# karenyang/GCN-VAE

Hardware: AMD Instinct MI355X
Metric: edges/sec R-GCN forward+backward, FB15k-237 emb=200 (higher is better)
Workload: dtype f32; 1 GPU; FB15k-237-shaped synthetic full graph (BASELINE configs[1]): 14541 entities, 474 directed relation types, E=544230 directed edges on this rank (544230 in the trained graph), 2-layer R-GCN-VAE bdd num_bases=100 emb_dim=200 dropout 0.2, 0 IAF blocks, DistMult decoder on T=220000 triplets per rank, step = fwd + loss(BCE+reg+KL+MMD) + bwd + clip + Adam; edges_per_gpu=544230, trained_graph_edges=544230, nodes=14541, triplets_per_gpu=220000, n_flows=0, gemm_precision=f32, launch=hipgraph, parallelism=single GPU, optimizer=replicated clip + Adam, k1_operands=f32

## Files before the change

### gcn-vae_amd/csrc/k_loss.hip

```cpp
#include "common.h"

namespace gv {

constexpr int RED_BLOCKS = 1024;

__device__ __forceinline__ float block_sum_256(float v, float* sm ) {
    v = wave_sum(v);
    const int lane = threadIdx.x & 63, w = threadIdx.x >> 6;
    __syncthreads();
    if (lane == 0) sm[w] = v;
    __syncthreads();
    return sm[0] + sm[1] + sm[2] + sm[3];
}

__global__ __launch_bounds__(256) void k_final_sum(const float* part, int n, float scale, float* out, int accumulate) {
    __shared__ float sm[4];
    float acc = 0.f;
    for (int i = threadIdx.x; i < n; i += 256) acc += part[i];
    const float tot = block_sum_256(acc, sm);
    if (threadIdx.x == 0) *out = accumulate ? *out + scale * tot : scale * tot;
}

__global__ __launch_bounds__(256) void k_loss_combine(const float* p0, int n0, float s0, const float* p1, int n1, float s1,
                                                      const float* p2, int n2, float s2, const float* p3, int n3, float s3,
// ... 984 lines not shown
    for (int g = 0; g < G; ++g) {
        float4 t;
        t.x = (rl_dyn(acc[g].x, l16) + rl_dyn(acc[g].x, 16 + l16)) + (rl_dyn(acc[g].x, 32 + l16) + rl_dyn(acc[g].x, 48 + l16));
        t.y = (rl_dyn(acc[g].y, l16) + rl_dyn(acc[g].y, 16 + l16)) + (rl_dyn(acc[g].y, 32 + l16) + rl_dyn(acc[g].y, 48 + l16));
        t.z = (rl_dyn(acc[g].z, l16) + rl_dyn(acc[g].z, 16 + l16)) + (rl_dyn(acc[g].z, 32 + l16) + rl_dyn(acc[g].z, 48 + l16));
        t.w = (rl_dyn(acc[g].w, l16) + rl_dyn(acc[g].w, 16 + l16)) + (rl_dyn(acc[g].w, 32 + l16) + rl_dyn(acc[g].w, 48 + l16));
        if (lane < 16) sm[w][l16 + 16 * g] = t;
    }
    __syncthreads();
    const bool indexed = !is_x && yidx;
    float* o = is_x ? gx + (size_t)row * h : gy + (size_t)(yidx ? yidx[row] : row) * h;
    for (int q = threadIdx.x; q < (h >> 2); q += 64 * MMD_WAVES) {
        float4 s4 = sm[0][q];
#pragma unroll
        for (int i = 1; i < MMD_WAVES; ++i) { const float4 t = sm[i][q]; s4.x += t.x; s4.y += t.y; s4.z += t.z; s4.w += t.w; }
        if (indexed) {
            atomicAdd(o + 4 * q, s4.x); atomicAdd(o + 4 * q + 1, s4.y); atomicAdd(o + 4 * q + 2, s4.z); atomicAdd(o + 4 * q + 3, s4.w);
        } else {
            *reinterpret_cast<float4*>(o + 4 * q) = s4;
        }
    }
}

__global__ __launch_bounds__(256) void k_prior_sample_fwd(const float* z_pre, const float* eps, float* out, int s, int k, int h) {
    const int total = s * h;
    for (int i = blockIdx.x * 256 + threadIdx.x; i < total; i += gridDim.x * 256) {
        const int r = i / h, c = i - r * h, j = r % k;
        const float v = softplus_t(z_pre[(size_t)(k + j) * h + c]) + 1e-8f;
        out[i] = z_pre[(size_t)j * h + c] + eps[i] * sqrtf(v);
    }
}

__global__ __launch_bounds__(256) void k_prior_sample_bwd(const float* z_pre, const float* eps, const float* g, float* gz_pre,
                                                          int accumulate, int s, int k, int h) {
    const int total = k * h;
    for (int i = blockIdx.x * 256 + threadIdx.x; i < total; i += gridDim.x * 256) {
        const int j = i / h, c = i - j * h;
        const float raw = z_pre[(size_t)(k + j) * h + c];
        const float v = softplus_t(raw) + 1e-8f;
        float gm = 0.f, gs = 0.f;
        for (int r = j; r < s; r += k) {
            gm += g[(size_t)r * h + c];
            gs += g[(size_t)r * h + c] * eps[(size_t)r * h + c];
        }
        const float gr = gs * 0.5f / sqrtf(v) * (raw > 20.f ? 1.f : 1.f / (1.f + expf(-raw)));
        gz_pre[i] = accumulate ? gz_pre[i] + gm : gm;
        gz_pre[total + i] = accumulate ? gz_pre[total + i] + gr : gr;
    }
}

struct DmFusedParams {
    const int4* items;
    int n_items;
    const int* rel_s;
    const int* rel_o;
    const int* rel_tid;
    const float* e;
    int ld_e;
    const float* w;
    int ld_w;
    const float* labels;
    const float* bias;
    const int* pos3;
    float* score;
    float* delta;
    float* u;
    float* partial;
    float* part;
    int h;
};

// ... 476 lines not shown
    static const int v2 = getenv("GV_MMD_ROWS16") ? atoi(getenv("GV_MMD_ROWS16")) : 1;
    const bool al = h % 4 == 0 && aligned16(x) && aligned16(y) && aligned16(gx) && aligned16(gy);
    if (v2 && al && h <= 256) hipLaunchKernelGGL(k_mmd_bwd_g<4>, dim3(sx + sy), dim3(64 * MMD_WAVES), 0, GV_ST, x, y, y_index, sx, sy, h, gmmd, gscale, gx, gy);
    else if (h <= 256) hipLaunchKernelGGL(k_mmd_bwd<4>, dim3(sx + sy), dim3(64 * MMD_WAVES), 0, GV_ST, x, y, y_index, sx, sy, h, gmmd, gscale, gx, gy);
    else hipLaunchKernelGGL(k_mmd_bwd<16>, dim3(sx + sy), dim3(64 * MMD_WAVES), 0, GV_ST, x, y, y_index, sx, sy, h, gmmd, gscale, gx, gy);
    return launch_status("gv_mmd_bwd");
}

extern "C" int gv_prior_sample_fwd(const float* z_pre, const float* eps, float* out, int s, int k, int h, void* stream) {
    GV_REQUIRE(z_pre && eps && out, GV_ERR_NULL, "gv_prior_sample_fwd: NULL pointer");
    GV_REQUIRE(s > 0 && k > 0 && h > 0, GV_ERR_SHAPE, "gv_prior_sample_fwd: bad shape");
    hipLaunchKernelGGL(k_prior_sample_fwd, dim3((s * h + 255) / 256), dim3(256), 0, GV_ST, z_pre, eps, out, s, k, h);
    return launch_status("gv_prior_sample_fwd");
}

extern "C" int gv_prior_sample_bwd(const float* z_pre, const float* eps, const float* g, float* gz_pre, int accumulate,
                                   int s, int k, int h, void* stream) {
    GV_REQUIRE(z_pre && eps && g && gz_pre, GV_ERR_NULL, "gv_prior_sample_bwd: NULL pointer");
    GV_REQUIRE(s > 0 && k > 0 && h > 0, GV_ERR_SHAPE, "gv_prior_sample_bwd: bad shape");
    hipLaunchKernelGGL(k_prior_sample_bwd, dim3((k * h + 255) / 256), dim3(256), 0, GV_ST, z_pre, eps, g, gz_pre, accumulate, s, k, h);
    return launch_status("gv_prior_sample_bwd");
}

extern "C" int gv_distmult_bce_fwd_grad(const int32_t* items, int n_items, const int32_t* rel_s, const int32_t* rel_o,
                                        const int32_t* rel_tid, const float* embed, int ld_e, const float* w_rel, int ld_w,
                                        const float* labels, const float* bias, const int32_t* pos3, float* score,
                                        float* delta, float* u, float* partial, float* workspace, int64_t t, int h,
                                        void* stream) {
    GV_REQUIRE(items && rel_s && rel_o && rel_tid && embed && w_rel && labels && score && delta && u && workspace,
               GV_ERR_NULL, "gv_distmult_bce_fwd_grad: NULL pointer");
    GV_REQUIRE(t > 0 && t < (1ll << 30) && n_items > 0, GV_ERR_SHAPE, "gv_distmult_bce_fwd_grad: t=%lld n_items=%d",
               (long long)t, n_items);
    GV_REQUIRE(h > 0 && h <= 256 && h % 4 == 0 && ld_e >= h && ld_w >= h && ld_e % 4 == 0 && ld_w % 4 == 0, GV_ERR_SHAPE,
               "gv_distmult_bce_fwd_grad: h=%d (ld %d, %d): the fused sweep covers h <= 256, h %% 4 == 0", h, ld_e, ld_w);
    GV_REQUIRE(aligned16(embed) && aligned16(w_rel) && aligned16(u) && aligned16(partial), GV_ERR_ALIGN,
               "gv_distmult_bce_fwd_grad: 16-B alignment required");
    DmFusedParams p{(const int4*)items, n_items, rel_s, rel_o, rel_tid, embed, ld_e, w_rel, ld_w, labels, bias, pos3,
                    score, delta, u, partial, workspace, h};
    hipLaunchKernelGGL(k_distmult_bce_fwd_grad<8>, dim3(red_blocks(t, 16)), dim3(256), 0, GV_ST, p);
    return launch_status("gv_distmult_bce_fwd_grad");
}

extern "C" int gv_distmult_grad_finish(const float* gloss, const float* u, const float* partial, const int32_t* fix,
                                       int n_fix, const int32_t* rowptr, int chunk, int num_rels, int h,
                                       const float* w_rel, int ld_w, float reg_scale, float* grad_w, int ld_gw,
                                       int accumulate, const float* delta, float* d_out, int64_t n_coef,
// ... 19 lines not shown
```

### gcn-vae_amd/encoders.py

```python
import random

import numpy as np
import torch
import torch.nn as nn
import torch.nn.functional as F

from . import ops, prob
from .flows import MADE, PermuteLayer
from .layers import RelGraphConv


class EmbeddingLayer(ops.StayOnDevice, nn.Module):
    def __init__(self, num_nodes, h_dim):
        super().__init__()
        self.embedding = nn.Embedding(num_nodes, h_dim)

    def forward(self, g, h, r, norm):
        h = ops.to_module_device(self.embedding.weight, h)
        return ops.embedding(self.embedding.weight, h.squeeze(), ops.device_rng(self.embedding.weight.device),
                             sole_consumer=True)


class DistLayer(ops.StayOnDevice, nn.Module):

# ... 49 lines not shown
        self.input_layer = EmbeddingLayer(self.num_nodes, self.h_dim)
        self.rconv_layer_1 = RelGraphConv(self.h_dim, self.h_dim, self.num_rels, "bdd", self.num_bases,
                                          activation=nn.ReLU(), self_loop=True, dropout=self.dropout)
        self.rconv_layer_2 = RelGraphConv(self.h_dim, self.h_dim * 2, self.num_rels, "bdd", self.num_bases,
                                          activation=None, self_loop=True, dropout=self.dropout)

    def sample_z(self, batch):
        m, v = prob.gaussian_parameters(self.z_pre.squeeze(0), dim=0)
        idx = torch.distributions.categorical.Categorical(self.pi).sample((batch,))
        x = prob.sample_gaussian(m[idx], v[idx])
        if self.n_flows > 0:
            for flow in self.nf[::-1]:
                x, _ = flow.inverse(x)
        return x

    def compute_kernel(self, x, y):
        dim = x.size(1)
        d2 = (x.unsqueeze(1) - y.unsqueeze(0)).pow(2).mean(2) / float(dim)
        return torch.exp(-d2)

    def get_kl(self, z):
        return ops.kl_to_mixture(z, self.z_mean, self.z_sigma, self.z_pre.squeeze(0), self.flow_log_prob)

    def _prior_draw(self, device, dtype):
        num_sample = 200
        rows = (num_sample // self.k) * self.k if num_sample // self.k > 1 else self.k
        if self.mmd_eps_override is not None:
            eps = self.mmd_eps_override
        elif self._prior_eps_next is not None:
            eps, self._prior_eps_next = self._prior_eps_next, None
        else:
            eps = torch.empty(rows, self.h_dim, device=device, dtype=dtype)
            ops.device_rng(device).fill([(eps, ops.RNG_NORMAL, 0.0, self.rng_stream_prior)])
        return ops.prior_sample(self.z_pre.squeeze(0), eps)

    def _prior_rows(self):
        num_sample = 200
        return (num_sample // self.k) * self.k if num_sample // self.k > 1 else self.k

    def _draw_noise(self, n, device):
        jobs, eps = [], self.eps_override
        for layer in (self.rconv_layer_1, self.rconv_layer_2):
            if layer.wants_keep_mask():
                layer._keep_next = torch.empty(n, layer.out_feat, dtype=torch.uint8, device=device)
                jobs.append(layer.keep_job(layer._keep_next))
        if eps is None:
            eps = torch.empty(n, self.h_dim, dtype=torch.float32, device=device)
            jobs.append((eps, ops.RNG_NORMAL, 0.0, self.rng_stream_eps))
        if self.batch_mmd_prior_with_forward and self.training and self.mmd_eps_override is None:
            self._prior_eps_next = torch.empty(self._prior_rows(), self.h_dim, dtype=torch.float32, device=device)
            jobs.append((self._prior_eps_next, ops.RNG_NORMAL, 0.0, self.rng_stream_prior))
        if jobs:
            ops.device_rng(device).fill(jobs)
        return eps

    def mmd_inputs(self, z):
        num_sample = 200
        if self._z_pri_flowed is not None:
            z_pri, self._z_pri_flowed = self._z_pri_flowed, None
        else:
            z_pri = self._prior_draw(z.device, z.dtype)
            if self.n_flows > 0:
                for flow in self.nf:
                    z_pri, _ = flow.forward(z_pri)
        if self.mmd_index_override is not None:
            pick = self.mmd_index_override
        elif self.row_part is not None and getattr(self.row_part, 'real_positions', None) is not None:
            real = self.row_part.real_positions
            pick = torch.as_tensor(real[random.sample(range(len(real)), num_sample)], device=z.device)
        else:
            pick = torch.tensor(random.sample(range(z.shape[0]), num_sample), device=z.device)
        return z_pri, pick

    def get_mmd(self, z):
        z_pri, pick = self.mmd_inputs(z)
        return ops.mmd(z_pri, ops.embedding(z, pick))

    def get_flow_log_prob(self):
        return self.flow_log_prob

    def _forward_rows(self, g, h, r, norm):
        from .distributed import AllGatherRows
        from .distributed import AllReduceSum
        part = self.row_part
# ... 130 lines not shown
```

### gcn-vae_amd/lib.py

```python
import ctypes
import os

import torch

_HERE = os.path.dirname(os.path.abspath(__file__))
LIB_PATH = os.path.join(_HERE, 'libgcnvae_hip.so')

_P, _I, _L, _F = ctypes.c_void_p, ctypes.c_int, ctypes.c_int64, ctypes.c_float

SIGNATURES = {
    'gv_version': (_I, []),
    'gv_last_error_string': (ctypes.c_char_p, []),
    'gv_index_caps': (None, [_L, _I, _I, _P, _P, _P]),
    'gv_index_workspace_bytes': (_L, [_L, _I]),
    'gv_build_csr': (_I, [_P, _L, _I, _I, _P, _P, _P, _I, _P, _I, _P, _L, _P]),
    'gv_build_csr_batch_workspace_bytes': (_L, [_P, _I]),
    'gv_build_csr_batch': (_I, [_P, _I, _P, _L, _P]),
    'gv_triplet_lists': (_I, [_P, _I, _L, _P, _P, _P, _P, _P, _P, _P, _P, _P]),
    'gv_widen2_i32': (_I, [_P, _P, _L, _P, _P, _L, _P]),
    'gv_graph_index_build': (_I, [_P, _P, _L, _I, _I, _I, _I, _P, _P, _P, _P, _I, _P, _I, _P, _P, _P, _P, _I, _P, _I, _P, _L, _P]),
    'gv_relation_index_build': (_I, [_P, _P, _P, _P, _P, _L, _I, _I, _P, _P, _P, _P, _P, _P, _P, _I, _P, _I, _P, _L, _P]),
    'gv_triplet_index_build': (_I, [_P, _L, _I, _I, _I, _I, _P, _P, _P, _P, _P, _I, _P, _I, _P, _P, _P, _P, _P, _I, _P, _I,
                                    _P, _L, _P]),
    'gv_perm_sample': (_I, [_L, _L, ctypes.c_uint64, ctypes.c_uint64, _P, _P, ctypes.c_uint32, _P, _P]),
# ... 107 lines not shown
    'gv_scatter_add_rows': (_I, [_P, _P, _P, _L, _I, _P]),
    'gv_reparam_fwd': (_I, [_P, _P, _P, _P, _P, _L, _I, _P]),
    'gv_reparam_bwd': (_I, [_P, _P, _P, _P, _P, _P, _P, _L, _I, _P]),
    'gv_distmult_bce_fwd': (_I, [_P, _I, _P, _I, _P, _P, _P, _P, _P, _P, _P, _L, _I, _P]),
    'gv_bce_grad': (_I, [_P, _P, _P, _P, _P, _P, _P, _P, _P, _L, _P]),
    'gv_distmult_bce_fwd_grad': (_I, [_P, _I, _P, _P, _P, _P, _I, _P, _I, _P, _P, _P, _P, _P, _P, _P, _P, _L, _I, _P]),
    'gv_distmult_grad_finish': (_I, [_P, _P, _P, _P, _I, _P, _I, _I, _I, _P, _I, _F, _P, _I, _I, _P, _P, _L, _P, _P, _L, _P]),
    'gv_mean_sq': (_I, [_P, _L, _F, _P, _P, _I, _P]),
    'gv_mean_sq2': (_I, [_P, _L, _F, _P, _L, _F, _P, _P, _P, _L, _P]),
    'gv_axpby': (_I, [_L, _P, _F, _P, _F, _P, _P]),
    'gv_mul': (_I, [_L, _P, _P, _P, _P]),
    'gv_mul_multi': (_I, [_I, _P, _P, _P, _P, _P]),
    'gv_kl_workspace_bytes': (_L, [_L, _I, _I]),
    'gv_kl_fwd': (_I, [_P, _P, _I, _P, _P, _P, _P, _P, _P, _L, _I, _I, _P, _P]),
    'gv_kl_bwd': (_I, [_P, _P, _I, _P, _P, _P, _P, _F, _F, _P, _P, _P, _P, _I, _P, _I, _L, _I, _I, _P, _P]),
    'gv_reparam_kl_fwd': (_I, [_P, _P, _P, _P, _P, _P, _P, _P, _L, _I, _I, _P]),
    'gv_reparam_kl_bwd': (_I, [_P, _P, _P, _P, _P, _P, _P, _F, _F, _P, _P, _P, _I, _P, _L, _I, _I, _P]),
    'gv_loss_combine': (_I, [_P, _L, _P, _L, _L, _P, _L, _I, _I, _P, _I, _I, _F, _F, _F, _P, _P, _P, _P]),
    'gv_lincomb4': (_I, [_P, _F, _P, _F, _P, _F, _P, _F, _P, _P]),
    'gv_mmd_fwd': (_I, [_P, _P, _P, _I, _I, _I, _P, _P, _P]),
    'gv_mmd_bwd': (_I, [_P, _P, _P, _I, _I, _I, _P, _F, _P, _P, _P]),
    'gv_prior_sample_fwd': (_I, [_P, _P, _P, _I, _I, _I, _P]),
    'gv_prior_sample_bwd': (_I, [_P, _P, _P, _P, _I, _I, _I, _I, _P]),
    'gv_iaf_update_fwd': (_I, [_P, _P, _I, _P, _P, _P, _L, _I, _P]),
    'gv_iaf_update_bwd': (_I, [_P, _P, _I, _P, _P, _P, _P, _P, _P, _L, _I, _P]),
    'gv_iaf_update_bwd_acc': (_I, [_P, _P, _I, _P, _P, _P, _P, _I, _P, _P, _L, _I, _P]),
    'gv_rowsum': (_I, [_P, _I, _I, _I, _P, _L, _P]),
    'gv_reverse_cols': (_I, [_P, _P, _L, _I, _P]),
    'gv_mean_rows_multi': (_I, [_I, _P, _L, _P, _P, _P, _P]),
    'gv_mean_rows_bwd': (_I, [_P, _L, _L, _P, _P, _P]),
    'gv_adam_step': (_I, [_P, _P, _P, _P, _L, _P, _F, _F, _F, _F, _F, _P, _P]),
    'gv_clip_adam_step': (_I, [_P, _P, _P, _P, _L, _P, _P, _F, _F, _F, _F, _F, _P, _I, _P]),
}

_lib = None
_fns = {}


def load():
    global _lib
    if _lib is None:
        if not os.path.exists(LIB_PATH):
            raise RuntimeError(
                f'{LIB_PATH} not found: the HIP extension is not built. Run `python gcn-vae_amd/_build.py` '
                '(or __graft_entry__.build()). There is no CPU fallback for this path.')
        lib = ctypes.CDLL(LIB_PATH)
# ... 53 lines not shown
```

### gcn-vae_amd/ops.py

```python
import contextlib
import ctypes as _ct
import itertools as _it
import os as _os
from dataclasses import dataclass
from typing import Optional

import torch

from . import lib
from .lib import ptr

ACT_NONE, ACT_RELU = 0, 1

DIRECT_GRAD = {}
GRAD_FRESH = set()
DIRECT_EPOCH = [0]


def _stamp_direct(ctx):
    ctx._gv_direct_epoch = DIRECT_EPOCH[0]


def _verify_direct(ctx):
    if getattr(ctx, '_gv_direct_epoch', DIRECT_EPOCH[0]) != DIRECT_EPOCH[0]:
# ... 2319 lines not shown
        out = torch.empty_like(eps)
        ctx.set_materialize_grads(False)
        lib.call('gv_prior_sample_fwd', ptr(z_pre), ptr(eps), ptr(out), eps.shape[0], k, h, lib.stream())
        ctx.save_for_backward(z_pre, eps)
        return out

    @staticmethod
    def backward(ctx, g):
        z_pre, eps = ctx.saved_tensors
        if g is None:
            return None, None
        g = _chk(g.contiguous(), name='g')
        d_zp = _direct_flat(z_pre)
        gz = d_zp if d_zp is not None else torch.empty_like(z_pre)
        lib.call('gv_prior_sample_bwd', ptr(z_pre), ptr(eps), ptr(g), ptr(gz), 1 if d_zp is not None else 0, eps.shape[0],
                 z_pre.shape[0] // 2, z_pre.shape[1], lib.stream())
        return (None if d_zp is not None else gz), None


def prior_sample(z_pre, eps):
    return _PriorSample.apply(z_pre, eps)


class _LossHead(torch.autograd.Function):

    @staticmethod
    def forward(ctx, z, z_mean, z_sigma, w_rel, z_pre, flp, z_pri, pick, labels, tidx, reg_w, kl_w, mmd_w, score_bias,
                embed_rows=None, rows_dev=None, kl_link=None, grad_mode=True):
        z, ld_z = _row_major(z, 'embed')
        if rows_dev is not None:
            rows_dev = _chk(rows_dev.reshape(-1), torch.int32, 'rows_dev')
            if kl_w <= 0 or embed_rows is not None:
                raise NotImplementedError('rows_dev needs kl_w > 0 (the padding rows are masked in the KL pass) and no embed_rows')
        w_rel, ld_w = _row_major(w_rel, 'w_relation')
        labels = _chk(labels.reshape(-1), name='labels')
        dev, (n, h), T = z.device, z.shape, tidx.T
        if labels.numel() != T:
            raise ValueError('labels / triplets length mismatch')
        f32 = dict(dtype=torch.float32, device=dev)
        ctx.set_materialize_grads(False)
        scal = torch.empty(4, **f32)
        pred, reg, kl, mmd = scal[0:1], scal[1:2], scal[2:3], scal[3:4]
        ws, ws2 = torch.empty(2048, **f32), torch.empty(1024, **f32)
        score = torch.empty(T, **f32)
        loss = torch.empty((), **f32)
        bias = flp if (score_bias and flp is not None) else None
        resp = wsk = z_post = wsm = None
        link = kl_link if (kl_link is not None and not kl_link.claimed and kl_w > 0 and flp is None and rows_dev is None
                           and embed_rows is None and kl_link.matches(z_pre) and kl_link.resp.shape[0] == n) else None
        if link is not None:
            link.claimed = True
        if kl_w > 0:
            z_mean, z_sigma = _chk(z_mean.contiguous(), name='z_mean'), _chk(z_sigma.contiguous(), name='z_sigma')
            z_pre = _chk(z_pre.contiguous(), name='z_pre')
            k = z_pre.shape[0] // 2
            if link is None:
                wsk = torch.empty(int(lib.load().gv_kl_workspace_bytes(n, h, k)) // 4, **f32)
                resp = torch.empty(n, k, **f32)
        if mmd_w > 0:
            z_pri = _chk(z_pri.contiguous(), name='z_pri')
            pick = _chk(pick.reshape(-1), torch.int64, 'pick')
            wsm = torch.empty(z_pri.shape[0] + pick.numel(), **f32)
        if ld_z != h or ld_w != h:
            raise ValueError('loss_head needs contiguous embeddings and relation table')
        st = lib.stream()
        if link is not None:
            resp, wsk = link.resp, link.ws
        elif kl_w > 0:
            lib.call('gv_kl_fwd', ptr(z), ptr(z_mean), h, ptr(z_sigma), ptr(z_pre), ptr(flp), ptr(resp), None, ptr(wsk),
                     n, h, k, ptr(rows_dev), st)
        if mmd_w > 0:
            lib.call('gv_mmd_fwd', ptr(z_pri), ptr(z), ptr(pick), z_pri.shape[0], pick.numel(), h, None, ptr(wsm), st)
        z_count = z.numel() if embed_rows is None else int(embed_rows) * h
        lib.call('gv_mean_sq2', ptr(z), z.numel(), 1.0 / z_count, ptr(w_rel), w_rel.numel(), 1.0 / w_rel.numel(), None,
                 ptr(ws2), ptr(rows_dev), n, st)
        ctx.fused = None
        if grad_mode and (ctx.needs_input_grad[0] or ctx.needs_input_grad[3]) and distmult_fused_ok(z, ld_z, w_rel, ld_w):
            ctx.fused = _distmult_fused_fwd(z, ld_z, w_rel, ld_w, labels, bias, tidx, score, ws)
            ctx.ws = ws
        else:
            lib.call('gv_distmult_bce_fwd', ptr(z), ld_z, ptr(w_rel), ld_w, ptr(tidx.trip32), ptr(tidx.fwd_order), ptr(labels),
                     ptr(bias), ptr(score), None, ptr(ws), T, h, st)
        lib.call('gv_loss_combine', ptr(ws), T, ptr(ws2), z.numel(), w_rel.numel(), ptr(wsk) if kl_w > 0 else None, n, h,
                 (z_pre.shape[0] // 2) if kl_w > 0 else 0, ptr(wsm) if mmd_w > 0 else None,
                 z_pri.shape[0] if mmd_w > 0 else 0, pick.numel() if mmd_w > 0 else 0, float(reg_w), float(kl_w),
                 float(mmd_w), ptr(scal), ptr(loss), ptr(rows_dev), st)
        ctx.save_for_backward(z, z_mean if kl_w > 0 else None, z_sigma if kl_w > 0 else None, w_rel,
                              z_pre if kl_w > 0 else None, resp, z_pri if mmd_w > 0 else None, z_post,
                              pick if mmd_w > 0 else None, labels, score, wsk, rows_dev)
        ctx.meta = (tidx, float(reg_w), float(kl_w), float(mmd_w), bias is not None, flp is not None and kl_w > 0)
        ctx.z_count = z_count
        ctx.kl_link = link
        ctx.direct_w = _direct(w_rel) if ld_w == h else None
        _stamp_direct(ctx)
        out_pred, out_kl, out_mmd = pred.reshape(()), kl.reshape(1), mmd.reshape(())
        ctx.mark_non_differentiable(out_pred, out_kl, out_mmd)
        return loss, out_pred, out_kl, out_mmd

    @staticmethod
    def backward(ctx, g, _gp, _gk, _gm):
        if g is None:
            return (None,) * 18
        z, z_mean, z_sigma, w_rel, z_pre, resp, z_pri, z_post, pick, labels, score, wsk, rows_dev = ctx.saved_tensors
        z_count = ctx.z_count
        tidx, reg_w, kl_w, mmd_w, has_bias, flp_in_kl = ctx.meta
        dev, (n, h), T = z.device, z.shape, tidx.T
        f32 = dict(dtype=torch.float32, device=dev)
        g = _chk(g.reshape(1).contiguous(), name='gloss')
        fused = ctx.fused
        dscore = torch.empty(T, **f32) if fused is None else None
        dbias = torch.empty((), **f32) if has_bias else None
        ws = torch.empty(1024, **f32) if fused is None else None
        link = ctx.kl_link
        gz = torch.empty_like(z) if link is None else None
        gm = gv = gzp = d_zp = g_pri = g_post = None
        if link is not None:
            link.gkl, link.gscale, link.z_extra = g, kl_w, 2.0 * reg_w / z_count
            d_zp = True
        elif kl_w > 0:
            k = z_pre.shape[0] // 2
            d_zp = _direct_flat(z_pre)
            gm, gv = torch.empty_like(z), torch.empty_like(z)
            gzp = d_zp if d_zp is not None else torch.empty_like(z_pre)
        if mmd_w > 0:
            g_pri = torch.empty_like(z_pri)
        _verify_direct(ctx)
        d_w = ctx.direct_w
        g_w = d_w if d_w is not None else torch.empty_like(w_rel)
        g_flp = torch.empty((), **f32) if (has_bias or flp_in_kl) else None
        st = lib.stream()
        with fork(1):
            s1 = lib.stream()
            if link is not None:
                pass
            elif kl_w > 0:
                lib.call('gv_kl_bwd', ptr(z), ptr(z_mean), h, ptr(z_sigma), ptr(z_pre), ptr(resp), ptr(g), kl_w,
                         2.0 * reg_w / z_count, ptr(gz), ptr(gm), ptr(gv), ptr(gzp), 1 if d_zp is not None else 0, ptr(wsk),
                         1, n, h, k, ptr(rows_dev), s1)
            else:
                lib.call('gv_axpby', z.numel(), ptr(g), 2.0 * reg_w / z_count, ptr(z), 0.0, ptr(gz), s1)
            if mmd_w > 0 and link is None:
                lib.call('gv_mmd_bwd', ptr(z_pri), ptr(z), ptr(pick), z_pri.shape[0], pick.numel(), h, ptr(g), mmd_w,
                         ptr(g_pri), ptr(gz), s1)
        if fused is not None:
            d_inc = _distmult_fused_finish(fused, g, tidx, w_rel, h, 2.0 * reg_w / w_rel.numel(), g_w, d_w is not None, ctx.ws,
                                           dbias)
            idx_inc = None if tidx.pos3 is not None else tidx.inc_tid
        else:
            if tidx.pos3 is not None:
                d_inc, d_rel, idx_inc, idx_rel = torch.empty(2 * T, **f32), torch.empty(T, **f32), None, None
            else:
                d_inc, d_rel, idx_inc, idx_rel = dscore, dscore, tidx.inc_tid, tidx.rel_tid
            lib.call('gv_bce_grad', ptr(score), ptr(labels), ptr(g), ptr(dscore), ptr(tidx.pos3),
                     ptr(d_inc) if tidx.pos3 is not None else None, ptr(d_rel) if tidx.pos3 is not None else None,
                     ptr(dbias), ptr(ws), T, st)
            bdd_grad_weight(tidx.rel, tidx.rel_s, tidx.rel_o, d_rel, idx_rel, z, z, h, 1, 1, out=g_w,
                            accumulate=d_w is not None)
            lib.call('gv_axpby', w_rel.numel(), ptr(g), 2.0 * reg_w / w_rel.numel(), ptr(w_rel), 1.0, ptr(g_w), st)
        join(1)
        g_z = bdd_aggregate(indices.largest_first(tidx.inc) if indices.K1_ITEMS_LARGEST_FIRST else tidx.inc, tidx.inc_other, tidx.inc_rel,
                            d_inc, idx_inc, z, w_rel, h, 1, 1, addend=gz)
        if link is not None and mmd_w > 0:
            lib.call('gv_mmd_bwd', ptr(z_pri), ptr(z), ptr(pick), z_pri.shape[0], pick.numel(), h, ptr(g), mmd_w,
                     ptr(g_pri), ptr(g_z), st)
        if g_flp is not None:
            lib.call('gv_lincomb4', ptr(dbias) if has_bias else None, 1.0, ptr(g) if flp_in_kl else None, kl_w, None, 0.0,
                     None, 0.0, ptr(g_flp), st)
        return (g_z, gm, gv, (None if d_w is not None else g_w), (None if d_zp is not None else gzp), g_flp, g_pri, None,
                None, None, None, None, None, None, None, None, None, None)


def loss_head(z, z_mean, z_sigma, w_rel, z_pre, flp, z_pri, pick, labels, tidx, reg_w, kl_w, mmd_w, score_bias,
              embed_rows=None, rows_dev=None):
    return _LossHead.apply(z, z_mean, z_sigma, w_rel, z_pre, flp, z_pri, pick, labels, tidx, float(reg_w), float(kl_w),
                           float(mmd_w), bool(score_bias), embed_rows, rows_dev, getattr(z, '_gv_kl_link', None),
                           torch.is_grad_enabled())


from .made import *
from .made import _ChainLayer, _RowLayer, _MADEForward, _MADEForwardBF16
from . import made


TRANSE_MAX_DIM = 512


def _i32(t, name, n=None):
    t = _chk(t, torch.int32, name)
    if not t.is_contiguous() or (n is not None and t.numel() != n):
        raise ValueError(f'{name}: expected a contiguous int32 tensor of {n} entries')
    return t


def _table(t, name):
    t = _chk(t, name=name)
    if t.dim() != 2 or not t.is_contiguous() or not 1 <= t.shape[1] <= TRANSE_MAX_DIM:
# ... 294 lines not shown
```

### gcn-vae_amd/train.py

```python
import argparse
import time

import numpy as np
import torch
import torch.nn as nn

from . import ops, ranking, sampling
from .optim import FlatAdam
from .data import load_data
from .encoders import KGVAE, RGCN
from .sampling import node_norm_to_edge_norm


class LinkPredict(ops.StayOnDevice, nn.Module):
    def __init__(self, model_class, in_dim, h_dim, num_rels, num_bases=-1, num_hidden_layers=1, dropout=0,
                 use_cuda=True, reg_param=0, kl_param=0, mmd_param=0, k=1, n_flows=0):
        super().__init__()
        self.encoder = model_class(num_nodes=in_dim, h_dim=h_dim, out_dim=h_dim, num_rels=num_rels * 2,
                                   num_bases=num_bases, num_hidden_layers=num_hidden_layers, dropout=dropout,
                                   use_self_loop=use_cuda, use_cuda=use_cuda, k=k, n_flows=n_flows)
        self.reg_param, self.kl_param, self.mmd_param = reg_param, kl_param, mmd_param
        if kl_param > 0 and hasattr(self.encoder, 'fuse_kl_with_reparam'):
            self.encoder.fuse_kl_with_reparam = True
        if mmd_param > 0 and hasattr(self.encoder, 'batch_mmd_prior_with_forward'):
# ... 8 lines not shown
        if key != self._tidx_key:
            self._tidx = ops.TripletIndex(triplets.to(embedding.device), embedding.shape[0], self.w_relation.shape[0],
                                          sync_free=not getattr(self, 'static_batch', False))
            self._tidx_key = key
            self._tidx_keepalive = triplets
        return self._tidx

    def calc_score(self, embedding, triplets):
        return ops.distmult_score(embedding, self.w_relation, self.triplet_index(embedding, triplets))

    def forward(self, g, h, r, norm):
        return self.encoder.forward(g, h, r, norm)

    def regularization_loss(self, embedding):
        return ops.mean_sq(embedding) + ops.mean_sq(self.w_relation)

    def get_loss(self, g, embed, triplets, labels):
        enc = self.encoder
        tidx = self.triplet_index(embed, triplets)
        vae = isinstance(enc, KGVAE)
        flp = enc.get_flow_log_prob() if vae else None
        kl_w = self.kl_param if vae else 0.0
        mmd_w = self.mmd_param if vae else 0.0
        z_pri, pick = enc.mmd_inputs(embed) if mmd_w > 0 else (None, None)
        part = getattr(enc, 'row_part', None) if vae else None
        if part is not None:
            return self._get_loss_rows(part, embed, tidx, flp, kl_w, mmd_w, z_pri, pick, labels)
        loss, predict_loss, kl, mmd = ops.loss_head(
            embed, enc.z_mean if kl_w > 0 else None, enc.z_sigma if kl_w > 0 else None, self.w_relation,
            enc.z_pre.squeeze(0) if kl_w > 0 else None, flp, z_pri, pick, labels, tidx, self.reg_param, kl_w, mmd_w,
            score_bias=self.n_flows > 0, rows_dev=getattr(self, 'rows_dev', None))
        kl = kl.reshape(()) if kl_w > 0 else kl.reshape(1)
        mmd = mmd.reshape(()) if mmd_w > 0 else mmd.reshape(1)
        if kl_w <= 0 or mmd_w <= 0:
            loss = loss.reshape(1)
        return loss, predict_loss, kl, mmd


def _get_loss_rows(self, part, embed, tidx, flp, kl_w, mmd_w, z_pri, pick, labels):
    enc = self.encoder
    head, predict_loss, _, mmd = ops.loss_head(embed, None, None, self.w_relation, None, flp, z_pri, pick, labels, tidx,
                                               self.reg_param, 0.0, mmd_w, score_bias=self.n_flows > 0,
                                               embed_rows=part.real_rows)
    kl = None
    if kl_w > 0 and part.own_rows > 0:
        kl = ops.kl_to_mixture(enc.z_own, enc.z_mean, enc.z_sigma, enc.z_pre.squeeze(0), flp)
    loss = ops.lincomb2(head, 1.0 / part.world, kl, kl_w * part.own_rows / max(part.real_rows, 1))
# ... 319 lines not shown
```

### include/gcnvae.h

```cpp
#ifndef GCNVAE_H
#define GCNVAE_H

#include <stdint.h>

#ifdef __cplusplus
extern "C" {
#endif

typedef enum {
    GV_OK = 0,
    GV_ERR_NULL = -1,
    GV_ERR_SHAPE = -2,
    GV_ERR_ALIGN = -3,
    GV_ERR_WORKSPACE = -4
} gv_status;

enum { GV_ACT_NONE = 0, GV_ACT_RELU = 1 };

int gv_version(void);
const char* gv_last_error_string(void);

int gv_segment_items_count(const int32_t* rowptr, int n_seg, int chunk, int32_t* n_chunks, int32_t* n_slots,
                           int32_t* is_split, void* stream);
int gv_segment_items_fill(const int32_t* rowptr, int n_seg, int chunk, const int32_t* item_off,
// ... 346 lines not shown
int gv_kl_bwd(const float* z, const float* m, int ld_m, const float* v, const float* z_pre, const float* resp,
              const float* gkl, float gscale, float z_extra, float* gz, float* gm, float* gv, float* g_zpre,
              int accumulate_zpre, float* workspace, int mix_ready, int64_t n, int h, int k, const int32_t* rows_dev,
              void* stream);
int gv_reparam_kl_fwd(const float* h2, const float* eps, const float* z_pre, float* z, float* v, float* m_out, float* resp,
                      float* workspace, int64_t n, int h, int k, void* stream);
int gv_reparam_kl_bwd(const float* z, const float* h2, const float* v, const float* eps, const float* z_pre, const float* resp,
                      const float* gkl, float gscale, float z_extra, const float* gz_up, float* gh2, float* g_zpre,
                      int accumulate_zpre, float* workspace, int64_t n, int h, int k, void* stream);

int gv_loss_combine(const float* ws_pred, int64_t t, const float* ws_reg, int64_t n_embed, int64_t n_wrel,
                    const float* ws_kl, int64_t n_nodes, int h, int k, const float* ws_mmd, int sx, int sy, float reg_w,
                    float kl_w, float mmd_w, float* scal , float* loss, const int32_t* rows_dev,
                    void* stream);
int gv_lincomb4(const float* a0, float c0, const float* a1, float c1, const float* a2, float c2, const float* a3,
                float c3, float* out, void* stream);
int gv_mmd_fwd(const float* x, const float* y, const int64_t* y_index, int sx, int sy, int h, float* mmd, float* workspace,
               void* stream);
int gv_mmd_bwd(const float* x, const float* y, const int64_t* y_index, int sx, int sy, int h, const float* gmmd, float gscale,
               float* gx, float* gy, void* stream);
int gv_prior_sample_fwd(const float* z_pre, const float* eps, float* out, int s, int k, int h, void* stream);
int gv_prior_sample_bwd(const float* z_pre, const float* eps, const float* g, float* gz_pre, int accumulate, int s, int k,
                        int h, void* stream);

int gv_iaf_update_fwd(const float* z, const float* net, int ld_net, const float* x_old, const int32_t* colcount,
                      float* x_new, int64_t n, int d, void* stream);
int gv_iaf_update_bwd(const float* z, const float* net, int ld_net, const int32_t* colcount, const float* g_xnew,
                      const float* g_logdet , float* g_z, float* g_net, float* g_xold, int64_t n, int d,
                      void* stream);
int gv_iaf_update_bwd_acc(const float* z, const float* net, int ld_net, const int32_t* colcount, const float* g_xnew,
                          const float* g_logdet, float* g_z, int gz_accumulate, float* g_net, float* g_xold, int64_t n, int d,
                          void* stream);
int gv_rowsum(const float* x, int ld, int col0, int ncols, float* out, int64_t n, void* stream);
int gv_reverse_cols(const float* x, float* out, int64_t n, int d, void* stream);
int gv_mean_rows_multi(int count, const float* const* x, int64_t n, const int32_t* rows_dev, float* out, float* workspace,
                       void* stream);
int gv_mean_rows_bwd(const float* g, int64_t len, int64_t n, const int32_t* rows_dev, float* out, void* stream);

int gv_adam_step(float* p, const float* g, float* exp_avg, float* exp_avg_sq, int64_t n, const float* sumsq,
                 float max_norm, float lr, float beta1, float beta2, float eps, const float* step, void* stream);
int gv_clip_adam_step(float* p, float* g, float* exp_avg, float* exp_avg_sq, int64_t n, float* workspace,
                      float* sumsq_out, float max_norm, float lr, float beta1, float beta2, float eps, float* step,
                      int zero_grad, void* stream);

void gv_index_caps(int64_t n_entries, int n_seg, int chunk, int* items_cap, int* fix_cap, int* slots_cap);
int64_t gv_index_workspace_bytes(int64_t n_entries, int n_seg_max);
// ... 63 lines not shown
```

Measured before the change: 569.4 million edges/s.

## Fuse prior sampling with MMD forward and gradient into one kernel pass

Defers the prior draw so that one kernel builds the prior samples from z_pre and eps and computes both the MMD value and per-row gradient directions in the forward pass. A small apply kernel then scales those directions by the upstream gradient and scatters them into the decoder and z_pre gradients. This removes the separate prior_sample forward/backward and MMD backward kernels and their passes over the pairwise rows. In exchange the forward always pays for the gradient work, adds buffers for u_pri and u_post, and only applies under a set of shape and alignment conditions.

```diff
diff --git a/gcn-vae_amd/csrc/k_loss.hip b/gcn-vae_amd/csrc/k_loss.hip
--- a/gcn-vae_amd/csrc/k_loss.hip
+++ b/gcn-vae_amd/csrc/k_loss.hip
@@ -1030,12 +1030,17 @@
     }
 }
 
+__device__ __forceinline__ float prior_sd(float raw) {
+    const float v = softplus_t(raw) + 1e-8f;
+    return sqrtf(v);
+}
+__device__ __forceinline__ float prior_elem(float mu, float e, float sd) { return mu + e * sd; }
+
 __global__ __launch_bounds__(256) void k_prior_sample_fwd(const float* z_pre, const float* eps, float* out, int s, int k, int h) {
     const int total = s * h;
     for (int i = blockIdx.x * 256 + threadIdx.x; i < total; i += gridDim.x * 256) {
         const int r = i / h, c = i - r * h, j = r % k;
-        const float v = softplus_t(z_pre[(size_t)(k + j) * h + c]) + 1e-8f;
-        out[i] = z_pre[(size_t)j * h + c] + eps[i] * sqrtf(v);
+        out[i] = prior_elem(z_pre[(size_t)j * h + c], eps[i], prior_sd(z_pre[(size_t)(k + j) * h + c]));
     }
 }
 
@@ -1055,6 +1060,145 @@
         gz_pre[i] = accumulate ? gz_pre[i] + gm : gm;
         gz_pre[total + i] = accumulate ? gz_pre[total + i] + gr : gr;
     }
+}
+
+template <int G>
+__global__ __launch_bounds__(64 * MMD_WAVES) void k_mmd_fwd_grad_g(const float* z_pre, const float* eps, int k, const float* y,
+                                                                    const int64_t* yidx, int sx, int sy, int h, float* z_pri,
+                                                                    float* part, float* u_pri, float* u_post) {
+    extern __shared__ __attribute__((aligned(16))) float4 smx[];
+    __shared__ float smt[MMD_WAVES];
+    const int lane = threadIdx.x & 63, l16 = lane & 15, w = threadIdx.x >> 6;
+    const int grp = (int)(threadIdx.x >> 4);
+    constexpr int NG = 4 * MMD_WAVES;
+    const int h4 = h >> 2, kh4 = k * h4;
+    float4* red = smx + 2 * kh4;
+    for (int i = threadIdx.x; i < kh4; i += 64 * MMD_WAVES) {
+        smx[i] = reinterpret_cast<const float4*>(z_pre)[i];
+        const float4 r4 = reinterpret_cast<const float4*>(z_pre)[kh4 + i];
+        smx[kh4 + i] = make_float4(prior_sd(r4.x), prior_sd(r4.y), prior_sd(r4.z), prior_sd(r4.w));
+    }
+    __syncthreads();
+    const bool is_x = (int)blockIdx.x < sx;
+    const int row = is_x ? blockIdx.x : blockIdx.x - sx;
+    bool on[G];
+    int col[G];
+#pragma unroll
+    for (int g = 0; g < G; ++g) { col[g] = 4 * (l16 + 16 * g); on[g] = col[g] < h; }
+    auto load_row = [&](bool from_y, int j, float4 (&v)[G]) {
+        if (from_y) {
+            mmd_load_row4<G>(y + (size_t)(yidx ? yidx[j] : j) * h, on, col, v);
+        } else {
+            const float* e = eps + (size_t)j * h;
+            const float4* mu = smx + (j % k) * h4;
+#pragma unroll
+            for (int g = 0; g < G; ++g) {
+                v[g] = make_float4(0.f, 0.f, 0.f, 0.f);
+                if (on[g]) {
+                    const float4 e4 = *reinterpret_cast<const float4*>(e + col[g]);
+                    const float4 m4 = mu[col[g] >> 2], s4 = mu[kh4 + (col[g] >> 2)];
+                    v[g] = make_float4(prior_elem(m4.x, e4.x, s4.x), prior_elem(m4.y, e4.y, s4.y), prior_elem(m4.z, e4.z, s4.z),
+                                       prior_elem(m4.w, e4.w, s4.w));
+                }
+            }
+        }
+    };
+    float4 av[G], acc[G];
+    load_row(!is_x, row, av);
+    if (is_x && threadIdx.x < 16) {
+#pragma unroll
+        for (int g = 0; g < G; ++g)
+            if (on[g]) *reinterpret_cast<float4*>(z_pri + (size_t)row * h + col[g]) = av[g];
+    }
+#pragma unroll
+    for (int g = 0; g < G; ++g) acc[g] = make_float4(0.f, 0.f, 0.f, 0.f);
+    const float inv = 1.f / ((float)h * (float)h);
+    const int n_same = is_x ? sx : sy, n_other = is_x ? sy : sx;
+    const float c_same = (-2.f * inv) * 2.f / ((float)n_same * (float)n_same);
+    const float c_other = (-2.f * inv) * (-2.f) / ((float)sx * (float)sy);
+    float tot = 0.f;
+    for (int pass = 0; pass < 2; ++pass) {
+        const bool b_is_y = pass == 0 ? !is_x : is_x;
+        const int nb = pass == 0 ? n_same : n_other;
+        const float cf = pass == 0 ? c_same : c_other;
+        const bool counts = pass == 0 || is_x;
+        const float wt = pass == 0 ? 1.f / ((float)nb * (float)nb) : -2.f / ((float)sx * (float)sy);
+        for (int j0 = 0; j0 < nb; j0 += 2 * NG) {
+            const int j = j0 + grp, j1 = j + NG;
+            float4 b0[G], b1[G];
+            load_row(b_is_y, min(j, nb - 1), b0);
+            load_row(b_is_y, min(j1, nb - 1), b1);
+            const float d0 = row16_sum(mmd_d2_4<G>(av, b0)), d1 = row16_sum(mmd_d2_4<G>(av, b1));
+            const float e0 = expf(-d0 * inv), e1 = expf(-d1 * inv);
+            if (counts) {
+                if (j < nb) tot += wt * e0;
+                if (j1 < nb) tot += wt * e1;
+            }
+            const float k0 = j < nb ? cf * e0 : 0.f, k1 = j1 < nb ? cf * e1 : 0.f;
+#pragma unroll
+            for (int g = 0; g < G; ++g) {
+                acc[g].x = fmaf(k0, av[g].x - b0[g].x, fmaf(k1, av[g].x - b1[g].x, acc[g].x));
+                acc[g].y = fmaf(k0, av[g].y - b0[g].y, fmaf(k1, av[g].y - b1[g].y, acc[g].y));
+                acc[g].z = fmaf(k0, av[g].z - b0[g].z, fmaf(k1, av[g].z - b1[g].z, acc[g].z));
+                acc[g].w = fmaf(k0, av[g].w - b0[g].w, fmaf(k1, av[g].w - b1[g].w, acc[g].w));
+            }
+        }
+    }
+    const float t = (rl_bcast_f(tot, 0) + rl_bcast_f(tot, 16)) + (rl_bcast_f(tot, 32) + rl_bcast_f(tot, 48));
+    if (lane == 0) smt[w] = t;
+#pragma unroll
+    for (int g = 0; g < G; ++g) {
+        float4 s;
+        s.x = (rl_dyn(acc[g].x, l16) + rl_dyn(acc[g].x, 16 + l16)) + (rl_dyn(acc[g].x, 32 + l16) + rl_dyn(acc[g].x, 48 + l16));
+        s.y = (rl_dyn(acc[g].y, l16) + rl_dyn(acc[g].y, 16 + l16)) + (rl_dyn(acc[g].y, 32 + l16) + rl_dyn(acc[g].y, 48 + l16));
+        s.z = (rl_dyn(acc[g].z, l16) + rl_dyn(acc[g].z, 16 + l16)) + (rl_dyn(acc[g].z, 32 + l16) + rl_dyn(acc[g].z, 48 + l16));
+        s.w = (rl_dyn(acc[g].w, l16) + rl_dyn(acc[g].w, 16 + l16)) + (rl_dyn(acc[g].w, 32 + l16) + rl_dyn(acc[g].w, 48 + l16));
+        if (lane < 16) red[w * 16 * G + l16 + 16 * g] = s;
+    }
+    __syncthreads();
+    if (threadIdx.x == 0) {
+        float s = 0.f;
+#pragma unroll
+        for (int i = 0; i < MMD_WAVES; ++i) s += smt[i];
+        part[blockIdx.x] = s;
+    }
+    float* o = (is_x ? u_pri : u_post) + (size_t)row * h;
+    for (int q = threadIdx.x; q < h4; q += 64 * MMD_WAVES) {
+        float4 s4 = red[q];
+#pragma unroll
+        for (int i = 1; i < MMD_WAVES; ++i) { const float4 x = red[i * 16 * G + q]; s4.x += x.x; s4.y += x.y; s4.z += x.z; s4.w += x.w; }
+        *reinterpret_cast<float4*>(o + 4 * q) = s4;
+    }
+}
+
+__global__ __launch_bounds__(256) void k_mmd_grad_apply(const float* u_pri, const float* u_post, const int64_t* pick,
+                                                        const float* z_pre, const float* eps, const float* gmmd, float gscale,
+                                                        float* gdec, int64_t n, float* gz_pre, int accumulate, int sx, int sy,
+                                                        int k, int h, int nb_post) {
+    const float c = gscale * (gmmd ? *gmmd : 1.f);
+    if ((int)blockIdx.x < nb_post) {
+        const int i = blockIdx.x * 256 + threadIdx.x;
+        if (i >= sy * h) return;
+        const int r = i / h, cc = i - r * h;
+        const int64_t dst = pick ? pick[r] : r;
+        if (dst >= 0 && dst < n) atomicAdd(gdec + dst * h + cc, c * u_post[i]);
+        return;
+    }
+    const int total = k * h;
+    const int i = ((int)blockIdx.x - nb_post) * 256 + threadIdx.x;
+    if (i >= total) return;
+    const int j = i / h, cc = i - j * h;
+    const float raw = z_pre[(size_t)(k + j) * h + cc];
+    const float v = softplus_t(raw) + 1e-8f;
+    float gm = 0.f, gs = 0.f;
+    for (int r = j; r < sx; r += k) {
+        const float g = c * u_pri[(size_t)r * h + cc];
+        gm += g;
+        gs += g * eps[(size_t)r * h + cc];
+    }
+    const float gr = gs * 0.5f / sqrtf(v) * (raw > 20.f ? 1.f : 1.f / (1.f + expf(-raw)));
+    gz_pre[i] = accumulate ? gz_pre[i] + gm : gm;
+    gz_pre[total + i] = accumulate ? gz_pre[total + i] + gr : gr;
 }
 
 struct DmFusedParams {
@@ -1577,6 +1721,34 @@
     return launch_status("gv_prior_sample_bwd");
 }
 
+extern "C" int gv_mmd_fused_ok(int h, int k) {
+    return h > 0 && k > 0 && h % 4 == 0 && h <= 256 && (int64_t)k * h <= 4096;
+}
+
+extern "C" int gv_mmd_fwd_grad(const float* z_pre, const float* eps, int k, const float* y, const int64_t* y_index, int sx, int sy,
+                               int h, float* z_pri, float* workspace, float* u_pri, float* u_post, void* stream) {
+    GV_REQUIRE(z_pre && eps && y && z_pri && workspace && u_pri && u_post, GV_ERR_NULL, "gv_mmd_fwd_grad: NULL pointer");
+    GV_REQUIRE(sx > 0 && sy > 0 && sx + sy <= RED_BLOCKS && gv_mmd_fused_ok(h, k), GV_ERR_SHAPE,
+               "gv_mmd_fwd_grad: sx=%d sy=%d h=%d k=%d (need h %% 4 == 0, h <= 256, k h <= 4096, sx+sy <= %d)", sx, sy, h, k, RED_BLOCKS);
+    GV_REQUIRE(aligned16(z_pre) && aligned16(eps) && aligned16(y) && aligned16(z_pri) && aligned16(u_pri) && aligned16(u_post),
+               GV_ERR_SHAPE, "gv_mmd_fwd_grad: rows must be 16-byte aligned");
+    const size_t lds = ((size_t)2 * k * (h / 4) + (size_t)MMD_WAVES * 16 * 4) * sizeof(float4);
+    hipLaunchKernelGGL(k_mmd_fwd_grad_g<4>, dim3(sx + sy), dim3(64 * MMD_WAVES), lds, GV_ST, z_pre, eps, k, y, y_index, sx, sy, h,
+                       z_pri, workspace, u_pri, u_post);
+    return launch_status("gv_mmd_fwd_grad");
+}
+
+extern "C" int gv_mmd_grad_apply(const float* u_pri, const float* u_post, const int64_t* pick, const float* z_pre, const float* eps,
+                                 const float* gmmd, float gscale, float* g_dec, int64_t n, float* gz_pre, int accumulate, int sx,
+                                 int sy, int k, int h, void* stream) {
+    GV_REQUIRE(u_pri && u_post && z_pre && eps && g_dec && gz_pre, GV_ERR_NULL, "gv_mmd_grad_apply: NULL pointer");
+    GV_REQUIRE(sx > 0 && sy > 0 && k > 0 && h > 0 && n > 0 && (pick || sy <= n), GV_ERR_SHAPE, "gv_mmd_grad_apply: bad shape");
+    const int nb_post = (sy * h + 255) / 256;
+    hipLaunchKernelGGL(k_mmd_grad_apply, dim3(nb_post + (k * h + 255) / 256), dim3(256), 0, GV_ST, u_pri, u_post, pick, z_pre, eps,
+                       gmmd, gscale, g_dec, n, gz_pre, accumulate, sx, sy, k, h, nb_post);
+    return launch_status("gv_mmd_grad_apply");
+}
+
 extern "C" int gv_distmult_bce_fwd_grad(const int32_t* items, int n_items, const int32_t* rel_s, const int32_t* rel_o,
                                         const int32_t* rel_tid, const float* embed, int ld_e, const float* w_rel, int ld_w,
                                         const float* labels, const float* bias, const int32_t* pos3, float* score,
diff --git a/gcn-vae_amd/encoders.py b/gcn-vae_amd/encoders.py
--- a/gcn-vae_amd/encoders.py
+++ b/gcn-vae_amd/encoders.py
@@ -95,7 +95,7 @@
     def get_kl(self, z):
         return ops.kl_to_mixture(z, self.z_mean, self.z_sigma, self.z_pre.squeeze(0), self.flow_log_prob)
 
-    def _prior_draw(self, device, dtype):
+    def _prior_draw(self, device, dtype, deferred=False):
         num_sample = 200
         rows = (num_sample // self.k) * self.k if num_sample // self.k > 1 else self.k
         if self.mmd_eps_override is not None:
@@ -105,7 +105,7 @@
         else:
             eps = torch.empty(rows, self.h_dim, device=device, dtype=dtype)
             ops.device_rng(device).fill([(eps, ops.RNG_NORMAL, 0.0, self.rng_stream_prior)])
-        return ops.prior_sample(self.z_pre.squeeze(0), eps)
+        return (ops.prior_draw if deferred else ops.prior_sample)(self.z_pre.squeeze(0), eps)
 
     def _prior_rows(self):
         num_sample = 200
@@ -127,12 +127,12 @@
             ops.device_rng(device).fill(jobs)
         return eps
 
-    def mmd_inputs(self, z):
+    def mmd_inputs(self, z, deferred=False):
         num_sample = 200
         if self._z_pri_flowed is not None:
             z_pri, self._z_pri_flowed = self._z_pri_flowed, None
         else:
-            z_pri = self._prior_draw(z.device, z.dtype)
+            z_pri = self._prior_draw(z.device, z.dtype, deferred and self.n_flows == 0)
             if self.n_flows > 0:
                 for flow in self.nf:
                     z_pri, _ = flow.forward(z_pri)
diff --git a/gcn-vae_amd/lib.py b/gcn-vae_amd/lib.py
--- a/gcn-vae_amd/lib.py
+++ b/gcn-vae_amd/lib.py
@@ -153,6 +153,9 @@
     'gv_mmd_bwd': (_I, [_P, _P, _P, _I, _I, _I, _P, _F, _P, _P, _P]),
     'gv_prior_sample_fwd': (_I, [_P, _P, _P, _I, _I, _I, _P]),
     'gv_prior_sample_bwd': (_I, [_P, _P, _P, _P, _I, _I, _I, _I, _P]),
+    'gv_mmd_fused_ok': (_I, [_I, _I]),
+    'gv_mmd_fwd_grad': (_I, [_P, _P, _I, _P, _P, _I, _I, _I, _P, _P, _P, _P, _P]),
+    'gv_mmd_grad_apply': (_I, [_P, _P, _P, _P, _P, _P, _F, _P, _L, _P, _I, _I, _I, _I, _I, _P]),
     'gv_iaf_update_fwd': (_I, [_P, _P, _I, _P, _P, _P, _L, _I, _P]),
     'gv_iaf_update_bwd': (_I, [_P, _P, _I, _P, _P, _P, _P, _P, _P, _L, _I, _P]),
     'gv_iaf_update_bwd_acc': (_I, [_P, _P, _I, _P, _P, _P, _P, _I, _P, _P, _L, _I, _P]),
diff --git a/gcn-vae_amd/ops.py b/gcn-vae_amd/ops.py
--- a/gcn-vae_amd/ops.py
+++ b/gcn-vae_amd/ops.py
@@ -2365,6 +2365,33 @@
     return _PriorSample.apply(z_pre, eps)
 
 
+MMD_FUSED = _os.environ.get('GV_MMD_FUSED', '1') == '1'
+
+
+class PriorDraw:
+    __slots__ = ('z_pre', 'eps', 'z_pri')
+
+    def __init__(self, z_pre, eps):
+        self.z_pre, self.eps, self.z_pri = z_pre, eps, None
+
+    def sample(self):
+        return prior_sample(self.z_pre, self.eps)
+
+    def fusable(self, z, z_pre, pick, mmd_w):
+        zp, eps = self.z_pre, self.eps
+        return (MMD_FUSED and mmd_w > 0 and torch.is_grad_enabled() and z_pre is not None and pick is not None
+                and zp.data_ptr() == z_pre.data_ptr() and zp.shape == z_pre.shape and zp.is_contiguous()
+                and z.dim() == 2 and z.is_contiguous() and zp.dim() == 2 and eps.dim() == 2 and eps.shape[1] == z.shape[1] == zp.shape[1]
+                and eps.is_contiguous() and zp.dtype == eps.dtype == z.dtype == torch.float32
+                and zp.data_ptr() % 16 == 0 and eps.data_ptr() % 16 == 0 and z.data_ptr() % 16 == 0
+                and eps.shape[0] + pick.numel() <= 1024
+                and bool(lib.load().gv_mmd_fused_ok(int(z.shape[1]), int(zp.shape[0] // 2))))
+
+
+def prior_draw(z_pre, eps):
+    return PriorDraw(z_pre, eps) if MMD_FUSED else prior_sample(z_pre, eps)
+
+
 class _LossHead(torch.autograd.Function):
 
     @staticmethod
@@ -2400,9 +2427,17 @@
             if link is None:
                 wsk = torch.empty(int(lib.load().gv_kl_workspace_bytes(n, h, k)) // 4, **f32)
                 resp = torch.empty(n, k, **f32)
+        draw = z_pri if isinstance(z_pri, PriorDraw) else None
+        eps_p = u_pri = u_post = None
         if mmd_w > 0:
-            z_pri = _chk(z_pri.contiguous(), name='z_pri')
             pick = _chk(pick.reshape(-1), torch.int64, 'pick')
+            if draw is None:
+                z_pri = _chk(z_pri.contiguous(), name='z_pri')
+            else:
+                z_pre = _chk(z_pre.contiguous(), name='z_pre')
+                eps_p = _chk(draw.eps, name='prior eps')
+                z_pri = torch.empty_like(eps_p)
+                u_pri, u_post = torch.empty_like(eps_p), torch.empty(pick.numel(), h, **f32)
             wsm = torch.empty(z_pri.shape[0] + pick.numel(), **f32)
         if ld_z != h or ld_w != h:
             raise ValueError('loss_head needs contiguous embeddings and relation table')
@@ -2412,7 +2447,11 @@
         elif kl_w > 0:
             lib.call('gv_kl_fwd', ptr(z), ptr(z_mean), h, ptr(z_sigma), ptr(z_pre), ptr(flp), ptr(resp), None, ptr(wsk),
                      n, h, k, ptr(rows_dev), st)
-        if mmd_w > 0:
+        if draw is not None:
+            lib.call('gv_mmd_fwd_grad', ptr(z_pre), ptr(eps_p), z_pre.shape[0] // 2, ptr(z), ptr(pick), eps_p.shape[0],
+                     pick.numel(), h, ptr(z_pri), ptr(wsm), ptr(u_pri), ptr(u_post), st)
+            draw.z_pri = z_pri
+        elif mmd_w > 0:
             lib.call('gv_mmd_fwd', ptr(z_pri), ptr(z), ptr(pick), z_pri.shape[0], pick.numel(), h, None, ptr(wsm), st)
         z_count = z.numel() if embed_rows is None else int(embed_rows) * h
         lib.call('gv_mean_sq2', ptr(z), z.numel(), 1.0 / z_count, ptr(w_rel), w_rel.numel(), 1.0 / w_rel.numel(), None,
@@ -2429,8 +2468,9 @@
                  z_pri.shape[0] if mmd_w > 0 else 0, pick.numel() if mmd_w > 0 else 0, float(reg_w), float(kl_w),
                  float(mmd_w), ptr(scal), ptr(loss), ptr(rows_dev), st)
         ctx.save_for_backward(z, z_mean if kl_w > 0 else None, z_sigma if kl_w > 0 else None, w_rel,
-                              z_pre if kl_w > 0 else None, resp, z_pri if mmd_w > 0 else None, z_post,
-                              pick if mmd_w > 0 else None, labels, score, wsk, rows_dev)
+                              z_pre if (kl_w > 0 or draw is not None) else None, resp,
+                              z_pri if (mmd_w > 0 and draw is None) else None, z_post,
+                              pick if mmd_w > 0 else None, labels, score, wsk, rows_dev, eps_p, u_pri, u_post)
         ctx.meta = (tidx, float(reg_w), float(kl_w), float(mmd_w), bias is not None, flp is not None and kl_w > 0)
         ctx.z_count = z_count
         ctx.kl_link = link
@@ -2444,7 +2484,9 @@
     def backward(ctx, g, _gp, _gk, _gm):
         if g is None:
             return (None,) * 18
-        z, z_mean, z_sigma, w_rel, z_pre, resp, z_pri, z_post, pick, labels, score, wsk, rows_dev = ctx.saved_tensors
+        z, z_mean, z_sigma, w_rel, z_pre, resp, z_pri, z_post, pick, labels, score, wsk, rows_dev, eps_p, u_pri, u_post = \
+            ctx.saved_tensors
+        mfused = u_pri is not None
         z_count = ctx.z_count
         tidx, reg_w, kl_w, mmd_w, has_bias, flp_in_kl = ctx.meta
         dev, (n, h), T = z.device, z.shape, tidx.T
@@ -2465,7 +2507,8 @@
             d_zp = _direct_flat(z_pre)
             gm, gv = torch.empty_like(z), torch.empty_like(z)
             gzp = d_zp if d_zp is not None else torch.empty_like(z_pre)
-        if mmd_w > 0:
+        gzp_m = None
+        if mmd_w > 0 and not mfused:
             g_pri = torch.empty_like(z_pri)
         _verify_direct(ctx)
         d_w = ctx.direct_w
@@ -2482,7 +2525,7 @@
                          1, n, h, k, ptr(rows_dev), s1)
             else:
                 lib.call('gv_axpby', z.numel(), ptr(g), 2.0 * reg_w / z_count, ptr(z), 0.0, ptr(gz), s1)
-            if mmd_w > 0 and link is None:
+            if mmd_w > 0 and link is None and not mfused:
                 lib.call('gv_mmd_bwd', ptr(z_pri), ptr(z), ptr(pick), z_pri.shape[0], pick.numel(), h, ptr(g), mmd_w,
                          ptr(g_pri), ptr(gz), s1)
         if fused is not None:
@@ -2503,18 +2546,29 @@
         join(1)
         g_z = bdd_aggregate(indices.largest_first(tidx.inc) if indices.K1_ITEMS_LARGEST_FIRST else tidx.inc, tidx.inc_other, tidx.inc_rel,
                             d_inc, idx_inc, z, w_rel, h, 1, 1, addend=gz)
-        if link is not None and mmd_w > 0:
+        if mfused:
+            tgt = gzp
+            if tgt is None:
+                tgt = _direct_flat(z_pre)
+                if tgt is None:
+                    tgt = gzp_m = torch.empty_like(z_pre)
+            lib.call('gv_mmd_grad_apply', ptr(u_pri), ptr(u_post), ptr(pick), ptr(z_pre), ptr(eps_p), ptr(g), mmd_w, ptr(g_z), n,
+                     ptr(tgt), 0 if gzp_m is not None else 1, eps_p.shape[0], pick.numel(), z_pre.shape[0] // 2, h, st)
+        elif link is not None and mmd_w > 0:
             lib.call('gv_mmd_bwd', ptr(z_pri), ptr(z), ptr(pick), z_pri.shape[0], pick.numel(), h, ptr(g), mmd_w,
                      ptr(g_pri), ptr(g_z), st)
         if g_flp is not None:
             lib.call('gv_lincomb4', ptr(dbias) if has_bias else None, 1.0, ptr(g) if flp_in_kl else None, kl_w, None, 0.0,
                      None, 0.0, ptr(g_flp), st)
-        return (g_z, gm, gv, (None if d_w is not None else g_w), (None if d_zp is not None else gzp), g_flp, g_pri, None,
+        g_zp = gzp_m if gzp_m is not None else (None if d_zp is not None else gzp)
+        return (g_z, gm, gv, (None if d_w is not None else g_w), g_zp, g_flp, g_pri, None,
                 None, None, None, None, None, None, None, None, None, None)
 
 
 def loss_head(z, z_mean, z_sigma, w_rel, z_pre, flp, z_pri, pick, labels, tidx, reg_w, kl_w, mmd_w, score_bias,
               embed_rows=None, rows_dev=None):
+    if isinstance(z_pri, PriorDraw) and not z_pri.fusable(z, z_pre, pick, float(mmd_w)):
+        z_pri = z_pri.sample() if mmd_w > 0 else None
     return _LossHead.apply(z, z_mean, z_sigma, w_rel, z_pre, flp, z_pri, pick, labels, tidx, float(reg_w), float(kl_w),
                            float(mmd_w), bool(score_bias), embed_rows, rows_dev, getattr(z, '_gv_kl_link', None),
                            torch.is_grad_enabled())
diff --git a/gcn-vae_amd/train.py b/gcn-vae_amd/train.py
--- a/gcn-vae_amd/train.py
+++ b/gcn-vae_amd/train.py
@@ -54,7 +54,7 @@
         flp = enc.get_flow_log_prob() if vae else None
         kl_w = self.kl_param if vae else 0.0
         mmd_w = self.mmd_param if vae else 0.0
-        z_pri, pick = enc.mmd_inputs(embed) if mmd_w > 0 else (None, None)
+        z_pri, pick = enc.mmd_inputs(embed, deferred=True) if mmd_w > 0 else (None, None)
         part = getattr(enc, 'row_part', None) if vae else None
         if part is not None:
             return self._get_loss_rows(part, embed, tidx, flp, kl_w, mmd_w, z_pri, pick, labels)
diff --git a/include/gcnvae.h b/include/gcnvae.h
--- a/include/gcnvae.h
+++ b/include/gcnvae.h
@@ -392,6 +392,12 @@
 int gv_prior_sample_fwd(const float* z_pre, const float* eps, float* out, int s, int k, int h, void* stream);
 int gv_prior_sample_bwd(const float* z_pre, const float* eps, const float* g, float* gz_pre, int accumulate, int s, int k,
                         int h, void* stream);
+int gv_mmd_fused_ok(int h, int k);
+int gv_mmd_fwd_grad(const float* z_pre, const float* eps, int k, const float* y, const int64_t* y_index, int sx, int sy, int h,
+                    float* z_pri, float* workspace, float* u_pri, float* u_post, void* stream);
+int gv_mmd_grad_apply(const float* u_pri, const float* u_post, const int64_t* pick, const float* z_pre, const float* eps,
+                      const float* gmmd, float gscale, float* g_dec, int64_t n, float* gz_pre, int accumulate, int sx, int sy,
+                      int k, int h, void* stream);
 
 int gv_iaf_update_fwd(const float* z, const float* net, int ld_net, const float* x_old, const int32_t* colcount,
                       float* x_new, int64_t n, int d, void* stream);
```

Result: no change. 574.3 million edges/s, median of 5 (+0.9%).
